# ml-rust/blazr

Measured on AMD Instinct MI355X. Metric: decode tokens/sec, Llama-3-8B AWQ-INT4 seq=1 on MI355X (and HBM-roofline fraction), higher is better.
Workload: dtype i4; 1 GPU; llama3-8b-awq greedy decode, batch 1, seq=1, prompt 16 (seed 26), whole step as one hipGraph; N>1 = independent replicas; resident_weight_bytes=5754585088, context_at_end=242

## Files before the change

### blazr_amd/csrc/bz_kernels.hip

```cpp
#include "bz_internal.h"
#include "bz_dev.h"
#include "bz_ggml.h"
#include <math.h>

#include <hip/hip_ext.h>

static thread_local BzTimingSink* g_sink = nullptr;
void bzk_set_timing_sink(BzTimingSink* s) { g_sink = s; }
BzTimingSink* bzk_timing_sink() { return g_sink; }

template <int NTH>
__device__ __forceinline__ void zero_duty(long long* zb, int zn) {
  if (zb)
    for (int i = blockIdx.x * NTH + threadIdx.x; i < zn; i += gridDim.x * NTH) zb[i] = 0;
}

template <int FIX>
__device__ __forceinline__ float vget(const void* p, int i, int act) {
  if (FIX) return round_act(fix2f(((const long long*)p)[i], act), act);
  return ((const float*)p)[i];
}

template <int FIX> struct RawT { typedef float T; };
template <> struct RawT<1> { typedef long long T; };
// ... 274 lines not shown
static size_t mlp_smem(int H) { return (size_t)(H >> 5) * XQ_NP * 16 + (size_t)(H >> 7) * 32 + 16 * 128 * 8 + 2 * XQ_NP * 16 + 32 + 16 * 8 + 64; }

bool bzk_mlp_fusable(const LinearDev& gu, const LinearDev& dn, int H, int I) {
  return gu.kind == LK_Q4G && dn.kind == LK_Q4G && !gu.perm && !dn.perm && gu.N == 2 * I && gu.K == H && dn.N == H && dn.K == I &&
         (H == 2048 || H == 4096) && I % 128 == 0 && mlp_smem(H) <= 64 * 1024;
}

int bzk_mlp_q4g(hipStream_t s, const LinearDev& gu, const LinearDev& dn, int H, int I, const Pro& pro, long long* acc, long long* zero_buf, int zero_n) {
  if (!bzk_mlp_fusable(gu, dn, H, I) || pro.act != BZ_F16) BZ_FAIL(BZ_E_INVALID, "fused MLP does not apply to this shape / activation dtype");
  const size_t smem = mlp_smem(H);
  const double bytes = (double)gu.algo_bytes + (double)dn.algo_bytes;
#define LAUNCH_MLP(FIX, GP, TP, W_) BZ_LAUNCH("mlp_q4g<norm+gate/up+silu+down>", bytes, (k_mlp_q4g<FIX, GP, TP, W_, BZ_F16>), dim3(I / 64), dim3(W_ * 64), smem, s, \
    (const uint4*)gu.w, (const __half*)gu.scales, (const unsigned char*)gu.zeros, gu.bias, (const uint4*)dn.w, (const __half*)dn.scales,            \
    (const unsigned char*)dn.zeros, dn.bias, H, I, pro, acc, zero_buf, zero_n)
  if (H == 4096) { if (pro.src.fix) LAUNCH_MLP(1, 2, 4, 16); else LAUNCH_MLP(0, 2, 4, 16); }
  else { if (pro.src.fix) LAUNCH_MLP(1, 2, 4, 8); else LAUNCH_MLP(0, 2, 4, 8); }
#undef LAUNCH_MLP
  BZ_HIP(hipGetLastError());
  return BZ_OK;
}

template <int MODE, int FIX, int MAXJ, int NPF>
__global__ __launch_bounds__(256) void k_gemv_q4g(const uint4* __restrict__ W, const __half* __restrict__ S,
                                                  const unsigned char* __restrict__ Z, const float* __restrict__ bias, int N, int K,
                                                  int GW, int nst, Pro pro, long long* acc, long long* zero_buf, int zero_n) {
  extern __shared__ __attribute__((aligned(16))) char smem[];
  const int KR = GW * 128;
  float* xs = (float*)smem;
  uint4* xpl = (uint4*)(xs + KR);
  int4* gpar = (int4*)(xpl + (KR >> 5) * XQ_NP);
  __half* sS = (__half*)(gpar + 2 * GW);
  unsigned char* sZ = (unsigned char*)(sS + 4 * GW * 64);
  float* red = (float*)(sZ + 4 * GW * 64);

  const int st = blockIdx.x % nst, ks = blockIdx.x / nst;
  const int wave = __builtin_amdgcn_readfirstlane(threadIdx.x >> 6), lane = threadIdx.x & 63;
  const int nt = st * 4 + wave;
  const bool wave_on = nt * 64 < N;
  const int G = K >> 7;
  const int k0 = ks * KR, g0 = ks * GW;

  zero_duty<256>(zero_buf, zero_n);

  const int ntc = wave_on ? nt : 0;
  unsigned sreg[8], zreg[4];
  {
    const unsigned* Sg = (const unsigned*)(S + ((size_t)ntc * G + g0) * 64);
    const unsigned* Zg = (const unsigned*)(Z + ((size_t)ntc * G + g0) * 64);
#pragma unroll
    for (int j = 0; j < 8; j++) sreg[j] = Sg[min(lane + 64 * j, GW * 32 - 1)];
#pragma unroll
    for (int j = 0; j < 4; j++) zreg[j] = Zg[min(lane + 64 * j, GW * 16 - 1)];
  }

  XRegs<MODE, FIX, MAXJ, Q4G_E> xr;
  xload<MODE, FIX, MAXJ, Q4G_E>(pro, k0, KR, xr);
  __builtin_amdgcn_sched_barrier(0);

  const uint4* wp = W + ((size_t)ntc * (K >> 5) + (k0 >> 5)) * 64 + lane;
  uint4 Wb[NPF][4];
#pragma unroll
  for (int b = 0; b < NPF; b++) {
    const int bc = min(b, GW - 1);
#pragma unroll
    for (int c = 0; c < 4; c++) Wb[b][c] = ldnt(wp + (bc * 4 + c) * 64);
  }

  xfinish<MODE, FIX, MAXJ, Q4G_E>(pro, KR, xr, xs, red, blockIdx.x == 0);
  {
    unsigned* sSw = (unsigned*)(sS + wave * GW * 64);
    unsigned* sZw = (unsigned*)(sZ + wave * GW * 64);
#pragma unroll
    for (int j = 0; j < 8; j++) if (lane + 64 * j < GW * 32) sSw[lane + 64 * j] = sreg[j];
#pragma unroll
    for (int j = 0; j < 4; j++) if (lane + 64 * j < GW * 16) sZw[lane + 64 * j] = zreg[j];
  }
  quant_x128<256>(xs, KR, xpl, gpar);
  __syncthreads();
  if (!wave_on) return;

  double y = 0.0;
  for (int gb = 0; gb < GW; gb += NPF) {
#pragma unroll
    for (int b = 0; b < NPF; b++) {
      const int g = gb + b;
      if (g < GW) {
        const float s = __half2float(sS[(wave * GW + g) * 64 + lane]);
        const int z = sZ[(wave * GW + g) * 64 + lane];
        q4g_consume(Wb[b], g, xpl, gpar, s, z, y);
        if (g + NPF < GW) {
#pragma unroll
          for (int c = 0; c < 4; c++) Wb[b][c] = ldnt(wp + ((g + NPF) * 4 + c) * 64);
        }
      }
    }
  }
  const int n = nt * 64 + lane;
  if (bias != nullptr && ks == 0) y += (double)bias[n];
  atomicAdd((unsigned long long*)(acc + n), (unsigned long long)d2fix(y, pro.act));
}

template <int FIX, int NJ, int ACT>
__global__ __launch_bounds__(768) void k_gemv_q4g_slim(const uint4* __restrict__ W, const __half* __restrict__ S, const unsigned char* __restrict__ Z,
                                                      const float* __restrict__ bias, int N, int H, Pro pro, long long* acc, long long* zero_buf, int zero_n) {
  __shared__ uint4 xpl[8 * XQ_NP];
  __shared__ int4 gpar[4];
  __shared__ double red[4];
  __shared__ unsigned cntv[2];
  volatile unsigned* cnt = cntv;
  const int tid = threadIdx.x, wave = __builtin_amdgcn_readfirstlane(tid >> 6), lane = tid & 63;
  const bool prolog = wave < 4;
  const int NKS = H >> 8, G = H >> 7;
  const int ksl = blockIdx.x % NKS, tg = blockIdx.x / NKS;
  asm volatile("" :: "s"(zero_buf), "s"(zero_n), "s"(acc), "s"(pro.h_in), "s"(pro.src.p), "s"(pro.norm_w), "s"(pro.h_out), "s"(pro.H),
               "s"(H), "s"(N), "s"(W), "s"(S), "s"(Z), "s"(bias));
  if (tid == 0) { cnt[0] = 0; cnt[1] = 0; }
  if (prolog) {
    const int pt = tid;
    const bool hasprev = pro.src.p != nullptr;
    const void* prevp = hasprev ? pro.src.p : (const void*)pro.h_in;
    float4 ha[NJ], hb[NJ];
    typename RawT<FIX>::T pv[NJ][8];
#pragma unroll
    for (int j = 0; j < NJ; j++) {
      const int i0 = (j * 256 + pt) * 8;
      ha[j] = *(const float4*)(pro.h_in + i0); hb[j] = *(const float4*)(pro.h_in + i0 + 4);
#pragma unroll
      for (int e = 0; e < 8; e++) pv[j][e] = vraw<FIX>(prevp, (FIX || hasprev) ? i0 + e : 0);
    }
    const int osl = 32 * ksl, jsel = osl >> 8, p0 = osl & 255;
    const bool mine = pt >= p0 && pt < p0 + 32;
    const int so = min(max(pt - p0, 0), 31);
    const float4 na = *(const float4*)(pro.norm_w + (osl + so) * 8), nb = *(const float4*)(pro.norm_w + (osl + so) * 8 + 4);
    __builtin_amdgcn_sched_barrier(0);
    __syncthreads();
    __builtin_amdgcn_sched_barrier(0);
    float v[NJ][8];
    double ssd = 0.0;
#pragma unroll
    for (int j = 0; j < NJ; j++) {
      const float t[8] = {ha[j].x, ha[j].y, ha[j].z, ha[j].w, hb[j].x, hb[j].y, hb[j].z, hb[j].w};
#pragma unroll
      for (int e = 0; e < 8; e++) v[j][e] = hasprev ? round_t<ACT>(t[e] + round_t<ACT>(FIX ? fix2f((long long)pv[j][e], ACT) : (float)pv[j][e])) : t[e];
#pragma unroll
      for (int e = 0; e < 8; e += 2) ssd += (double)(v[j][e] * v[j][e]) + (double)(v[j][e + 1] * v[j][e + 1]);
      if (blockIdx.x == 0 && pro.h_out) {
        const int i0 = (j * 256 + pt) * 8;
        *(float4*)(pro.h_out + i0) = make_float4(v[j][0], v[j][1], v[j][2], v[j][3]); *(float4*)(pro.h_out + i0 + 4) = make_float4(v[j][4], v[j][5], v[j][6], v[j][7]);
      }
    }
    ssd = wave_sum_d(ssd);
    if (lane == 0) { red[wave] = ssd; __builtin_amdgcn_s_waitcnt(0xc07f); atomicAdd((unsigned*)&cnt[0], 1u); }
    if (p0 / 64 == wave) {
      lds_wait_count(&cnt[0], 4);
      const float ss = (float)((red[0] + red[1]) + (red[2] + red[3]));
      const float rs = rms_scale(ss, (float)H, pro.eps);
      float sv[8];
#pragma unroll
      for (int e = 0; e < 8; e++) {
        sv[e] = v[0][e];
#pragma unroll
        for (int j = 1; j < NJ; j++) sv[e] = (j == jsel) ? v[j][e] : sv[e];
      }
      const float nwv[8] = {na.x, na.y, na.z, na.w, nb.x, nb.y, nb.z, nb.w};
      float x[8];
      float am = 0.f;
#pragma unroll
      for (int e = 0; e < 8; e++) { x[e] = mine ? round_t<ACT>(nwv[e] * round_t<ACT>(sv[e] * rs)) : 0.f; am = fmaxf(am, fabsf(x[e])); }
      am = grp_reduce<16, OpMax>(am);
      unsigned w[XQ_NP]; int sp[XQ_NP]; float cs;
      xq_split8(x, am, w, sp, cs);
#pragma unroll
      for (int p = 0; p < XQ_NP; p++) sp[p] = grp_reduce<16, OpAdd>(sp[p]);
      const int4 g2w = xq_gpar_hi<16>(w, sp);
      if (mine) {
        unsigned* plw = (unsigned*)xpl + ((so >> 2) * XQ_NP) * 4 + (so & 3);
#pragma unroll
        for (int p = 0; p < XQ_NP; p++) plw[p * 4] = w[p];
        if ((so & 15) == 0) {
          gpar[2 * (so >> 4)] = make_int4(__float_as_int(cs), sp[0], sp[1], sp[2]);
          gpar[2 * (so >> 4) + 1] = g2w;
        }
      }
      __builtin_amdgcn_s_waitcnt(0xc07f);
      if (lane == 0) atomicAdd((unsigned*)&cnt[1], 1u);
    }
    return;
  }
  const int tq = tg * 8 + (wave - 4);
  const bool q_on = tq * 64 < N;
  const int tqc = q_on ? tq : 0;
  const uint4* wq = W + ((size_t)tqc * (H >> 5) + ksl * 8) * 64 + lane;
  uint4 Q[8]; float sq[2]; int zq[2];
  __syncthreads();
  __builtin_amdgcn_sched_barrier(0);
#pragma unroll
  for (int c = 0; c < 8; c++) Q[c] = ldnt(wq + c * 64);
#pragma unroll
  for (int b = 0; b < 2; b++) { const size_t ix = ((size_t)tqc * G + ksl * 2 + b) * 64 + lane; sq[b] = __half2float(S[ix]); zq[b] = Z[ix]; }
  if (zero_buf)
    for (int i = blockIdx.x * 512 + (tid - 256); i < zero_n; i += gridDim.x * 512) zero_buf[i] = 0;
  lds_wait_count(&cnt[1], 1);
  if (q_on) {
    double y = 0.0;
#pragma unroll
    for (int b = 0; b < 2; b++) {
      if (b == 0) q4g_consume_at<0, 4>(Q, 0, 0, xpl, gpar, sq[0], zq[0], y);
      else q4g_consume_at<4, 4>(Q, 4, 2, xpl, gpar, sq[1], zq[1], y);
    }
    const int n = tq * 64 + lane;
    if (bias != nullptr && ksl == 0) y += (double)bias[n];
    atomicAdd((unsigned long long*)(acc + n), (unsigned long long)d2fix(y, ACT));
  }
}

template <int XDT>
__global__ __launch_bounds__(512) void k_gemm_q4g_rows(const uint4* __restrict__ W, const __half* __restrict__ S, const unsigned char* __restrict__ Z,
                                                      const float* __restrict__ bias, int N, int K, const unsigned short* __restrict__ X, int rows,
                                                      long long* __restrict__ acc) {
  __shared__ __attribute__((aligned(16))) float xs[8 * 256];
  __shared__ uint4 xpl[8 * 8 * XQ_NP];
  __shared__ int4 gpar[8 * 4];
  const int tid = threadIdx.x, wave = __builtin_amdgcn_readfirstlane(tid >> 6), lane = tid & 63;
  const int NKS = K >> 8, G = K >> 7;
  const int ksl = blockIdx.x % NKS, tq = (blockIdx.x / NKS) * 8 + wave;
  const bool q_on = tq * 64 < N;
  const int tqc = q_on ? tq : 0;
  const int xr = tid >> 6;
  const uint2 xraw = *(const uint2*)(X + (size_t)min(xr, rows - 1) * K + ksl * 256 + lane * 4);
  __builtin_amdgcn_sched_barrier(0);
  uint4 Q[2][4]; float sq[2]; int zq[2];
  {
    const uint4* wq = W + ((size_t)tqc * (K >> 5) + ksl * 8) * 64 + lane;
#pragma unroll
    for (int b = 0; b < 2; b++)
#pragma unroll
      for (int c = 0; c < 4; c++) Q[b][c] = ldnt(wq + (b * 4 + c) * 64);
#pragma unroll
    for (int b = 0; b < 2; b++) { const size_t ix = ((size_t)tqc * G + ksl * 2 + b) * 64 + lane; sq[b] = __half2float(S[ix]); zq[b] = Z[ix]; }
  }
  {
    const unsigned u[2] = {xraw.x, xraw.y};
    float v[4];
#pragma unroll
    for (int i = 0; i < 2; i++) {
      if (XDT == BZ_F16) { v[2 * i] = __half2float(__ushort_as_half((unsigned short)(u[i] & 0xffffu))); v[2 * i + 1] = __half2float(__ushort_as_half((unsigned short)(u[i] >> 16))); }
      else { v[2 * i] = __uint_as_float(u[i] << 16); v[2 * i + 1] = __uint_as_float(u[i] & 0xffff0000u); }
    }
    const bool on = xr < rows;
    *(float4*)(xs + xr * 256 + lane * 4) = on ? make_float4(v[0], v[1], v[2], v[3]) : make_float4(0.f, 0.f, 0.f, 0.f);
  }
  __syncthreads();
  quant_x128<512>(xs, 8 * 256, xpl, gpar);
  __syncthreads();
  if (!q_on) return;
  const int n = tq * 64 + lane;
  const double bv = (bias != nullptr && ksl == 0) ? (double)bias[n] : 0.0;
#pragma unroll
  for (int r = 0; r < 8; r++) {
    if (r < rows) {
      double y = bv;
      q4g_consume(Q[0], r * 2, xpl, gpar, sq[0], zq[0], y);
      q4g_consume(Q[1], r * 2 + 1, xpl, gpar, sq[1], zq[1], y);
      atomicAdd((unsigned long long*)(acc + (size_t)r * N + n), (unsigned long long)d2fix(y, XDT));
    }
  }
}

__global__ void k_fix_rows_finish(long long* acc, size_t n, int act, float* out) {
  for (size_t i = (size_t)blockIdx.x * blockDim.x + threadIdx.x; i < n; i += (size_t)gridDim.x * blockDim.x) { out[i] = round_act(fix2f(acc[i], act), act); acc[i] = 0; }
}

bool bzk_gemm_q4g_rows_ok(const LinearDev& L) { return L.kind == LK_Q4G && !L.perm && L.K % 256 == 0 && L.N % 64 == 0; }

int bzk_gemm_q4g_rows(hipStream_t s, const LinearDev& L, int xdt, const void* x16, int rows, int act, long long* acc, float* y) {
  if (!bzk_gemm_q4g_rows_ok(L) || (xdt != BZ_F16 && xdt != BZ_BF16) || xdt != act) BZ_FAIL(BZ_E_UNSUPPORTED, "gemm_q4g_rows: unsupported weight / activation format");
  const int nks = L.K / 256, ntg = (L.N / 64 + 7) / 8;
  for (int r0 = 0; r0 < rows; r0 += 8) {
    const int nr = std::min(8, rows - r0);
    const unsigned short* xp = (const unsigned short*)x16 + (size_t)r0 * L.K;
    const double bytes = (double)L.algo_bytes;
    if (xdt == BZ_F16) BZ_LAUNCH("gemm_q4g_rows", bytes, k_gemm_q4g_rows<BZ_F16>, dim3(nks * ntg), dim3(512), 0, s, (const uint4*)L.w, (const __half*)L.scales,
                                 (const unsigned char*)L.zeros, L.bias, L.N, L.K, xp, nr, acc);
    else BZ_LAUNCH("gemm_q4g_rows", bytes, k_gemm_q4g_rows<BZ_BF16>, dim3(nks * ntg), dim3(512), 0, s, (const uint4*)L.w, (const __half*)L.scales,
                   (const unsigned char*)L.zeros, L.bias, L.N, L.K, xp, nr, acc);
    hipLaunchKernelGGL(k_fix_rows_finish, dim3(std::min<size_t>(1024, ((size_t)nr * L.N + 255) / 256)), dim3(256), 0, s, acc, (size_t)nr * L.N, act, y + (size_t)r0 * L.N);
  }
  BZ_HIP(hipGetLastError());
  return BZ_OK;
}

bool bzk_gemv_slim_ok(const LinearDev& L, const Pro& pro) {
  static const bool off = getenv("BZ_NO_SLIM_QKV") != nullptr;
  return !off && L.kind == LK_Q4G && !L.perm && pro.mode == PRO_NORM && pro.perm == nullptr && L.K == pro.H && (L.K == 2048 || L.K == 4096 || L.K == 8192) && L.N % 64 == 0 &&
         L.N <= 16384;
}

enum { GQ_Q80 = 0, GQ_Q4K = 1, GQ_Q6K = 2, GQ_MIX = 3, GQ_Q5K = 4, GQ_Q40 = 5, GQ_Q41 = 6, GQ_Q50 = 7, GQ_Q51 = 8 };
__host__ __device__ constexpr bool gq_legacy(int f) { return f == GQ_Q40 || f == GQ_Q41 || f == GQ_Q50 || f == GQ_Q51; }
__host__ __device__ constexpr bool gq_has5(int f) { return f == GQ_Q50 || f == GQ_Q51; }
__host__ __device__ constexpr bool gq_affine(int f) { return f == GQ_Q41 || f == GQ_Q51; }
#define XQ_MAX 8355000.0f

template <int FMT>
__device__ __forceinline__ void quant8_x32(const float (&v)[8], int e0, bool on, int lane, unsigned* xh, unsigned* xm, unsigned* xl, int4* cpar, int4* cpar6 = nullptr) {
  float am = 0.f;
#pragma unroll
  for (int i = 0; i < 8; i++) am = fmaxf(am, fabsf(v[i]));
  am = grp_reduce<4, OpMax>(am);
  const float inv = am > 0.f ? XQ_MAX / am : 0.f;
  unsigned wh[2] = {0, 0}, wm[2] = {0, 0}, wl[2] = {0, 0};
  int sa[3] = {0, 0, 0}, sb[3] = {0, 0, 0};
  int ta[3] = {0, 0, 0}, tb[3] = {0, 0, 0};
#pragma unroll
  for (int i = 0; i < 8; i++) {
    const int xi = (int)rintf(v[i] * inv);
    const int lo = ((xi + 128) & 255) - 128;
    const int r1 = (xi - lo) >> 8;
    const int mid = ((r1 + 128) & 255) - 128;
    const int hi = (r1 - mid) >> 8;
    wh[i >> 2] |= ((unsigned)hi & 255u) << (8 * (i & 3));
    wm[i >> 2] |= ((unsigned)mid & 255u) << (8 * (i & 3));
    wl[i >> 2] |= ((unsigned)lo & 255u) << (8 * (i & 3));
    if (FMT == GQ_Q4K || FMT == GQ_MIX) { sa[0] += hi; sa[1] += mid; sa[2] += lo; if (i >= 4) { sb[0] += hi; sb[1] += mid; sb[2] += lo; } }
    if (FMT == GQ_Q6K || FMT == GQ_Q5K || gq_legacy(FMT)) { sa[0] += hi; sa[1] += mid; sa[2] += lo; }
  }
  if (FMT == GQ_Q6K || FMT == GQ_MIX) {
    const bool second = (lane & 2) != 0;
#pragma unroll
    for (int q = 0; q < 3; q++) {
      const int mine = sa[q] + dpp_get<DPP_XOR1>(sa[q]);
      const int other = dpp_get<DPP_XOR2>(mine);
      ta[q] = second ? other : mine;
      tb[q] = second ? mine : other;
    }
    if (FMT == GQ_Q6K) {
#pragma unroll
      for (int q = 0; q < 3; q++) { sa[q] = ta[q]; sb[q] = tb[q]; }
    }
  }
  if (FMT == GQ_Q4K || FMT == GQ_MIX) {
#pragma unroll
    for (int q = 0; q < 3; q++) {
      sa[q] = grp_reduce<4, OpAdd>(sa[q]);
      sb[q] = grp_reduce<4, OpAdd>(sb[q]);
    }
  }
  if (FMT == GQ_Q5K || gq_legacy(FMT)) {
#pragma unroll
    for (int q = 0; q < 3; q++) sa[q] = grp_reduce<4, OpAdd>(sa[q]);
  }
  if (on) {
    *(uint2*)(xh + e0 / 4) = make_uint2(wh[0], wh[1]);
    *(uint2*)(xm + e0 / 4) = make_uint2(wm[0], wm[1]);
    *(uint2*)(xl + e0 / 4) = make_uint2(wl[0], wl[1]);
    if ((lane & 3) == 0) {
      cpar[2 * (e0 >> 5)] = make_int4(__float_as_int(am * (1.0f / XQ_MAX)), sa[0], sa[1], sa[2]);
      cpar[2 * (e0 >> 5) + 1] = make_int4(sb[0], sb[1], sb[2], 0);
      if (FMT == GQ_MIX) {
        cpar6[2 * (e0 >> 5)] = make_int4(__float_as_int(am * (1.0f / XQ_MAX)), ta[0], ta[1], ta[2]);
        cpar6[2 * (e0 >> 5) + 1] = make_int4(tb[0], tb[1], tb[2], 0);
      }
// ... 2019 lines not shown

template <int HD, int KVDT, int WIN = 0>
__global__ __launch_bounds__(256) void k_attn_decode(AttnArgs a) {
  extern __shared__ __attribute__((aligned(16))) char smem[];
  constexpr int half = HD / 2;
  constexpr int LDR = HD + 4;
  const int rep = a.nq / a.nkv;
  float* qs = (float*)smem;
  float* knew = qs + HD;
  float* vnew = knew + HD;
  float* wred = vnew + HD;
  float* ored = wred + 8;
  const int hq = blockIdx.x, kvh = hq / rep;
  const int tid = threadIdx.x, wave = __builtin_amdgcn_readfirstlane(tid >> 6), lane = tid & 63;
  const int pos = a.pos[0];
  const int len = a.q_only ? pos : pos + 1;
  const int ncache = pos;
  const int lo = WIN ? att_lo(len, a.window) : 0;
  const KvView& kv = a.kv;
  zero_duty<256>(a.zero_buf, a.zero_n);

  if (!a.q_only) {
    const float* cr = a.cos_t + (size_t)pos * half;
    const float* sr = a.sin_t + (size_t)pos * half;
    for (int idx = tid; idx < 2 * half; idx += 256) {
      const int hh = idx / half, i = idx % half;
      const int base = hh == 0 ? hq * HD : a.nq * HD + kvh * HD;
      const int ia = a.interleaved ? 2 * i : i, ib = a.interleaved ? 2 * i + 1 : i + half;
      const float x0 = vsrc_get(a.qkv, base + ia, a.act), x1 = vsrc_get(a.qkv, base + ib, a.act);
      const float c = cr[i], s = sr[i];
      const float y0 = round_act(rope_lo(x0, x1, c, s), a.act), y1 = round_act(rope_hi(x0, x1, c, s), a.act);
      if (hh == 0) { qs[ia] = y0; qs[ib] = y1; }
      else { knew[ia] = y0; knew[ib] = y1; }
    }
    for (int i = tid; i < HD; i += 256) vnew[i] = vsrc_get(a.qkv, a.nq * HD + a.nkv * HD + kvh * HD + i, a.act);
    __syncthreads();
    if (hq % rep == 0) {
      size_t woff;
      if (kv.paged) woff = kv_slot_off(kv, a.layer, kvh, kv.slot ? kv.slot[0] : (kv.block_table[pos / kv.bs] * kv.bs + pos % kv.bs));
      else woff = kv_row_off(kv, a.layer, kvh, pos);
      for (int i = tid; i < HD; i += 256) { kv_st(kv.k, woff + i, kv.dtype, knew[i]); kv_st(kv.v, woff + i, kv.dtype, vnew[i]); }
    }
  } else {
    for (int i = tid; i < HD; i += 256) qs[i] = ((const float*)a.qkv.p)[hq * HD + i];
    __syncthreads();
  }

  const float scale = div_rn(1.0f, sqrt_rn((float)HD));
  float m = -INFINITY, l = 0.f;
  float o[HD];
#pragma unroll
  for (int i = 0; i < HD; i++) o[i] = 0.f;
  for (int p = lo + tid; p < len; p += 256) {
    KvRow<HD, KVDT> kr, vr;
    const size_t ro = p < ncache ? kv_row_off(kv, a.layer, kvh, p) : 0;
    if (p < ncache) kr.load(kv.k, ro); else kr.from_f32(knew);
    if (KVDT != BZ_F32) { if (p < ncache) vr.load(kv.v, ro); else vr.from_f32(vnew); }
    float d = 0.f;
#pragma unroll
    for (int i = 0; i < HD; i += 4) {
      const float4 qa = *(const float4*)(qs + i);
      d += kr.get(i) * qa.x + kr.get(i + 1) * qa.y + kr.get(i + 2) * qa.z + kr.get(i + 3) * qa.w;
    }
    if (KVDT == BZ_F32) { if (p < ncache) vr.load(kv.v, ro); else vr.from_f32(vnew); }
    const float s = d * scale;
    if (m == -INFINITY) {
      m = s; l = 1.f;
#pragma unroll
      for (int i = 0; i < HD; i++) o[i] = vr.get(i);
    } else {
      const float mn = fmaxf(m, s);
      const float alpha = bz_expf(m - mn), e = bz_expf(s - mn);
      l = l * alpha + e;
      m = mn;
#pragma unroll
      for (int i = 0; i < HD; i++) o[i] = o[i] * alpha + e * vr.get(i);
    }
  }
  const float wm = wave_max(m);
  if (lane == 0) wred[wave] = wm;
  __syncthreads();
  const float M = fmaxf(fmaxf(wred[0], wred[1]), fmaxf(wred[2], wred[3]));
  const float w = (m == -INFINITY) ? 0.f : bz_expf(m - M);
  const float ws = wave_sum(l * w);
  if (lane == 0) wred[4 + wave] = ws;
  const int nrows = min(len - lo, 256);
  if (tid < nrows) {
#pragma unroll
    for (int i = 0; i < HD; i += 4) *(float4*)(ored + tid * LDR + i) = make_float4(o[i] * w, o[i + 1] * w, o[i + 2] * w, o[i + 3] * w);
  }
  __syncthreads();
  const float inv = div_rn(1.0f, (wred[4] + wred[5]) + (wred[6] + wred[7]));
  constexpr int PH = 256 / HD;
  const int col = tid % HD, ph = tid / HD;
  float acc = 0.f;
  for (int r = ph; r < nrows; r += PH) acc += ored[r * LDR + col];
  __syncthreads();
  ored[ph * LDR + col] = acc;
  __syncthreads();
  if (tid < HD) {
    float t = 0.f;
#pragma unroll
    for (int q = 0; q < PH; q++) t += ored[q * LDR + tid];
    a.out[(size_t)hq * HD + tid] = round_act(t * inv, a.act);
  }
}


template <int KVDT, int FUSE, int TPW, int NW, int PAGED, int HD = 128, int WIN = 0>
__global__ __launch_bounds__(NW * 64) void k_attn2(AttnArgs a, const uint4* __restrict__ W, const __half* __restrict__ S,
                                               const unsigned char* __restrict__ Z, const float* __restrict__ bias, int CS, long long* acc) {
  static_assert(HD == 128 || (HD == 64 && FUSE != 1), "head_dim 128, or 64 without the int4 o_proj");
  constexpr int half = HD / 2, NPC = HD / 8, RPL = 64 / NPC, PW = 256 / NW, NL = PW / RPL, OW = NW > 8 ? 8 : NW, NTH = NW * 64;
  asm volatile("" :: "s"(a.zero_buf), "s"(a.zero_n), "s"(a.kv.k), "s"(a.kv.v), "s"(a.kv.cap), "s"(a.kv.layer_stride), "s"(a.layer), "s"(a.act),
               "s"(a.interleaved), "s"(a.rope_cur), "s"(a.qkv.p), "s"(a.qkv.fix), "s"(a.nq), "s"(a.nkv), "s"(a.q_only), "s"(a.pos), "s"(W), "s"(S),
               "s"(Z), "s"(bias), "s"(CS), "s"(acc), "s"(a.out), "s"(a.kv.bs), "s"(a.kv.n_kv));
  extern __shared__ __attribute__((aligned(16))) char smem[];
  unsigned* q2 = (unsigned*)smem;
  unsigned* k2 = q2 + 64;
  unsigned* v2 = k2 + 64;
  double* pout = (double*)(v2 + 64);
  double* lred = pout + NW * 128;
  float* wred = (float*)(lred + NW);
  float* outh = wred + 2 * NW;
  uint4* xpl = (uint4*)(outh + 128);
  int4* gpar = (int4*)(xpl + 4 * XQ_NP);
  const int rep = a.nq / a.nkv;
  const int hq = FUSE ? blockIdx.x / CS : blockIdx.x, cs = FUSE ? blockIdx.x % CS : 0, kvh = hq / rep;
  const int tid = threadIdx.x, wave = __builtin_amdgcn_readfirstlane(tid >> 6), lane = tid & 63;
  const int piece = lane % NPC, rsub = lane / NPC;
  const KvView& kv = a.kv;
  const int pos_v = a.pos[0];
  const int slot_v = PAGED ? *(kv.slot ? kv.slot : a.pos) : 0;
  const int fixq = a.q_only ? 0 : a.qkv.fix;
  int i0, i1;
  {
    const int hh = tid / half, i = tid % half;
    const int base = hh == 0 ? hq * HD : a.nq * HD + kvh * HD;
    const int ia = a.interleaved ? 2 * i : i, ib = a.interleaved ? 2 * i + 1 : i + half;
    const int vb = a.nq * HD + a.nkv * HD + kvh * HD + 2 * i;
    i0 = hh < 2 ? base + ia : vb; i1 = hh < 2 ? base + ib : vb + 1;
    if (a.q_only) { i0 = hq * HD + 2 * i; i1 = i0 + 1; }
    if (hh > 2) { i0 = 0; i1 = 0; }
  }
  unsigned r0l, r0h, r1l, r1h;
  vsrc_issue(a.qkv.p, fixq, i0, r0l, r0h);
  vsrc_issue(a.qkv.p, fixq, i1, r1l, r1h);
  const float* rc = a.q_only ? (const float*)a.qkv.p : a.rope_cur;
  const float pc = rc[tid % half], ps = rc[half + tid % half];
  if (a.zero_buf) {
    const int nblk = FUSE ? a.nq * CS : a.nq;
    for (int i = blockIdx.x * NTH + tid; i < a.zero_n; i += nblk * NTH) a.zero_buf[i] = 0;
  }
  uint4 Wb[FUSE == 1 ? TPW : 1][4];
  const int t0 = (cs * OW + wave % OW) * TPW;
  constexpr int DLD = FUSE == 2 ? TPW : 1;
  uint4 Wd[DLD];
  const int nd0 = (cs * NW + wave) * DLD * RPL;
  if (FUSE == 2) {
    const int K = a.nq * HD;
    const unsigned short* wd = (const unsigned short*)W;
#pragma unroll
    for (int t = 0; t < DLD; t++) Wd[t] = ldnt((const uint4*)(wd + (size_t)(nd0 + t * RPL + rsub) * K + hq * HD + piece * 8));
  }
  if (FUSE == 1) {
    const int K = a.nq * HD;
#pragma unroll
    for (int t = 0; t < TPW; t++) {
      const uint4* wp = W + ((size_t)(t0 + t) * (K >> 5) + hq * 4) * 64 + lane;
#pragma unroll
      for (int c = 0; c < 4; c++) Wb[t][c] = ldnt(wp + c * 64);
    }
  }
  __builtin_amdgcn_sched_barrier(0);
  const int pos = __builtin_amdgcn_readfirstlane(pos_v);
  const int pmax = pos > 0 ? pos - 1 : 0;
  const int len = a.q_only ? pos : pos + 1;
  const int lo = WIN ? att_lo(len, a.window) : 0, cb = WIN ? (lo & ~255) : 0;
  const unsigned short* kb0 = (const unsigned short*)kv.k + (size_t)a.layer * kv.layer_stride;
  const unsigned short* vb0 = (const unsigned short*)kv.v + (size_t)a.layer * kv.layer_stride;
  uint4 kr[NL], vr[NL];
#pragma unroll
  for (int i = 0; i < NL; i++) { kr[i] = make_uint4(0, 0, 0, 0); vr[i] = make_uint4(0, 0, 0, 0); }
#define ATT_ROW(i) (((i) * NW + wave) * RPL + rsub)
#define ATT_LIVE(c0_, i) ((c0_) + ((i) * NW + wave) * RPL < len)
  if (cb + wave * RPL < len) {
    if (!PAGED) {
      const unsigned short* kb = kb0 + (size_t)kvh * kv.cap * HD;
      const unsigned short* vb = vb0 + (size_t)kvh * kv.cap * HD;
#pragma unroll
      for (int i = 0; i < NL; i++) {
        if (ATT_LIVE(cb, i)) {
          const unsigned off = (unsigned)min(cb + ATT_ROW(i), pmax) * HD + piece * 8;
          kr[i] = *(const uint4*)(kb + off);
          vr[i] = *(const uint4*)(vb + off);
        }
      }
    } else {
      int blk[NL];
#pragma unroll
      for (int i = 0; i < NL; i++) blk[i] = ATT_LIVE(cb, i) ? kv.block_table[min(cb + ATT_ROW(i), pmax) / kv.bs] : 0;
#pragma unroll
      for (int i = 0; i < NL; i++) {
        if (ATT_LIVE(cb, i)) {
          const int pp = min(cb + ATT_ROW(i), pmax);
          const size_t off = (((size_t)blk[i] * kv.n_kv + kvh) * kv.bs + (pp % kv.bs)) * HD + piece * 8;
          kr[i] = *(const uint4*)(kb0 + off);
          vr[i] = *(const uint4*)(vb0 + off);
        }
      }
    }
  }
  const float px0 = vsrc_finish(fixq, r0l, r0h, a.act), px1 = vsrc_finish(fixq, r1l, r1h, a.act);
  if (!a.q_only) {
    if (tid < 2 * half) {
      const int hh = tid / half, i = tid % half;
      const int ia = a.interleaved ? 2 * i : i, ib = a.interleaved ? 2 * i + 1 : i + half;
      const float y0 = round_act(rope_lo(px0, px1, pc, ps), a.act), y1 = round_act(rope_hi(px0, px1, pc, ps), a.act);
      unsigned short* dst = (unsigned short*)(hh == 0 ? q2 : k2);
      const unsigned p0 = pack2<KVDT>(y0, y1);
      dst[ia] = (unsigned short)(p0 & 0xffffu);
      dst[ib] = (unsigned short)(p0 >> 16);
    } else if (tid < 3 * half) {
      v2[tid - 2 * half] = pack2<KVDT>(px0, px1);
    }
    __syncthreads();
    if (hq % rep == 0 && cs == 0 && tid < half) {
      size_t woff;
      if (PAGED) woff = kv_slot_off(kv, a.layer, kvh, kv.slot ? slot_v : (kv.block_table[pos / kv.bs] * kv.bs + pos % kv.bs));
      else woff = kv_row_off_t<0>(kv, a.layer, kvh, pos);
      ((unsigned*)((unsigned short*)kv.k + woff))[tid] = k2[tid];
      ((unsigned*)((unsigned short*)kv.v + woff))[tid] = v2[tid];
    }
  } else {
    if (tid < half) q2[tid] = pack2<KVDT>(px0, px1);
    __syncthreads();
  }

  const float scale = div_rn(1.0f, sqrt_rn((float)HD));
  const uint4 qq = ((const uint4*)q2)[piece];
  float qf[8];
  unpack2<KVDT>(qq.x, qf[0], qf[1]); unpack2<KVDT>(qq.y, qf[2], qf[3]); unpack2<KVDT>(qq.z, qf[4], qf[5]); unpack2<KVDT>(qq.w, qf[6], qf[7]);
  const bool single = len - cb <= 256;
  float sc_[NL];
  float Mw = -INFINITY;
#define ATT_SCORES(c0_)                                                                                                    \
  _Pragma("unroll") for (int i = 0; i < NL; i++) {                                                                         \
    if (!ATT_LIVE(c0_, i)) { sc_[i] = -INFINITY; continue; }                                                               \
    const int p = (c0_) + ATT_ROW(i);                                                                                      \
    uint4 kk = kr[i];                                                                                                      \
    if (!a.q_only && p == pos) { kk = ((const uint4*)k2)[piece]; vr[i] = ((const uint4*)v2)[piece]; }                      \
    float kf[8];                                                                                                           \
    unpack2<KVDT>(kk.x, kf[0], kf[1]); unpack2<KVDT>(kk.y, kf[2], kf[3]); unpack2<KVDT>(kk.z, kf[4], kf[5]); unpack2<KVDT>(kk.w, kf[6], kf[7]); \
    double d = 0.0;                                                                                                        \
    _Pragma("unroll") for (int e = 0; e < 8; e++) d = fma((double)kf[e], (double)qf[e], d);                                \
    d = grp_sum_d<NPC>(d);                                                                                                 \
    sc_[i] = (p < len && (!WIN || p >= lo)) ? (float)d * scale : -INFINITY;                                                \
  }
  for (int c0 = cb; c0 < len; c0 += 256) {
    const bool won = c0 + wave * RPL < len;
    if (!won) continue;
    if (c0 > cb) {
#pragma unroll
      for (int i = 0; i < NL; i++)
        if (ATT_LIVE(c0, i)) kr[i] = *(const uint4*)(kb0 + kv_row_off_t<PAGED>(kv, 0, kvh, min(c0 + ATT_ROW(i), pmax)) + piece * 8);
    }
    ATT_SCORES(c0)
#pragma unroll
    for (int i = 0; i < NL; i++) Mw = fmaxf(Mw, sc_[i]);
  }
  Mw = wave_max(Mw);
  if (lane == 0) wred[wave] = Mw;
  __syncthreads();
  float Mall = wred[0];
#pragma unroll
  for (int w = 1; w < NW; w++) Mall = fmaxf(Mall, wred[w]);
  double accv[8] = {0.0, 0.0, 0.0, 0.0, 0.0, 0.0, 0.0, 0.0};
  double lsum = 0.0;
  for (int c0 = cb; c0 < len; c0 += 256) {
    const bool won = c0 + wave * RPL < len;
    if (!won) continue;
    if (!single) {
#pragma unroll
      for (int i = 0; i < NL; i++) {
        if (ATT_LIVE(c0, i)) {
          const size_t off = kv_row_off_t<PAGED>(kv, 0, kvh, min(c0 + ATT_ROW(i), pmax)) + piece * 8;
          kr[i] = *(const uint4*)(kb0 + off);
          vr[i] = *(const uint4*)(vb0 + off);
        }
      }
      ATT_SCORES(c0)
    }
#pragma unroll
    for (int i = 0; i < NL; i++) {
      if (!ATT_LIVE(c0, i)) continue;
      const float e = (sc_[i] == -INFINITY) ? 0.f : bz_expf(sc_[i] - Mall);
      const double ed = (double)e;
      lsum += ed;
      float v[8];
      unpack2<KVDT>(vr[i].x, v[0], v[1]); unpack2<KVDT>(vr[i].y, v[2], v[3]);
      unpack2<KVDT>(vr[i].z, v[4], v[5]); unpack2<KVDT>(vr[i].w, v[6], v[7]);
#pragma unroll
      for (int q = 0; q < 8; q++) accv[q] = fma(ed, (double)v[q], accv[q]);
    }
  }
#undef ATT_SCORES
#undef ATT_LIVE
#undef ATT_ROW
  if (NPC == 8) lsum += dpp_get<DPP_ROR8>(lsum);
  lsum = xrow32_d(xrow16_d(lsum));
#pragma unroll
  for (int q = 0; q < 8; q++) {
    if (NPC == 8) accv[q] += dpp_get<DPP_ROR8>(accv[q]);
    accv[q] = xrow32_d(xrow16_d(accv[q]));
  }
  if (lane < NPC) {
#pragma unroll
    for (int q = 0; q < 8; q++) pout[wave * HD + piece * 8 + q] = accv[q];
  }
  if (lane == 0) lred[wave] = lsum;
  __syncthreads();
  float Orun = 0.f, Lrun = 1.f;
  if (tid < HD) {
    double oc = 0.0, Lc = 0.0;
#pragma unroll
    for (int w = 0; w < NW; w++) { oc += pout[w * HD + tid]; Lc += lred[w]; }
    Orun = (float)oc; Lrun = (float)Lc;
  }
  if (!FUSE) {
    if (tid < HD) a.out[(size_t)hq * HD + tid] = round_act(div_rn(Orun, Lrun), a.act);
    return;
  }
  if (tid < HD) outh[tid] = round_act(div_rn(Orun, Lrun), a.act);
  if (FUSE == 2) {
    __syncthreads();
    const float4 oa = *(const float4*)(outh + piece * 8), ob = *(const float4*)(outh + piece * 8 + 4);
    const float of8[8] = {oa.x, oa.y, oa.z, oa.w, ob.x, ob.y, ob.z, ob.w};
#pragma unroll
    for (int t = 0; t < DLD; t++) {
      float w8[8];
      unpack2<KVDT>(Wd[t].x, w8[0], w8[1]); unpack2<KVDT>(Wd[t].y, w8[2], w8[3]); unpack2<KVDT>(Wd[t].z, w8[4], w8[5]); unpack2<KVDT>(Wd[t].w, w8[6], w8[7]);
      double d = 0.0;
#pragma unroll
      for (int e = 0; e < 8; e++) d += (double)__fmul_rn(w8[e], of8[e]);
      d = grp_sum_d<NPC>(d);
      const int n = nd0 + t * RPL + rsub;
      if (piece == 0) {
        if (bias != nullptr && hq == 0) d += (double)bias[n];
        atomicAdd((unsigned long long*)(acc + n), (unsigned long long)d2fix(d, a.act));
      }
    }
    return;
  }
  float sc[FUSE == 1 ? TPW : 1]; int zp[FUSE == 1 ? TPW : 1];
  {
    const int G = (a.nq * HD) >> 7;
#pragma unroll
    for (int t = 0; t < (FUSE == 1 ? TPW : 1); t++) {
      sc[t] = __half2float(S[((size_t)(t0 + t) * G + hq) * 64 + lane]);
      zp[t] = Z[((size_t)(t0 + t) * G + hq) * 64 + lane];
    }
  }
  __syncthreads();
  quant_x128<NW * 64>(outh, HD, xpl, gpar);
  __syncthreads();
#pragma unroll
  for (int t = 0; t < (FUSE == 1 ? TPW : 1); t++) {
    double y = 0.0;
    q4g_consume(Wb[t], 0, xpl, gpar, sc[t], zp[t], y);
    const int n = (t0 + t) * 64 + lane;
    if (bias != nullptr && hq == 0) y += (double)bias[n];
    if (wave < OW) atomicAdd((unsigned long long*)(acc + n), (unsigned long long)d2fix(y, a.act));
  }
}


template <int PAGED, int FUSE = 0, int WIN = 0>
__global__ __launch_bounds__(512) void k_attn2f(AttnArgs a, const uint4* __restrict__ Wq, const uint4* __restrict__ Hd, const float* __restrict__ bias, int CS, long long* acc) {
  constexpr int HD = 128, half = 64, NW = 8, PW = 256 / NW, NL = PW / 4, NTH = NW * 64;
  __shared__ __attribute__((aligned(16))) float qf[HD], kf[HD], vf[HD];
  __shared__ float wred[2 * NW];
  __shared__ __attribute__((aligned(16))) float pout[NW * 128];
  __shared__ __attribute__((aligned(16))) float outh[FUSE ? HD : 4];
  __shared__ __attribute__((aligned(16))) unsigned xh[FUSE ? 32 : 4], xm[FUSE ? 32 : 4], xl[FUSE ? 32 : 4];
  __shared__ int4 cpar[FUSE ? 8 : 1];
  asm volatile("" :: "s"(a.zero_buf), "s"(a.zero_n), "s"(a.kv.k), "s"(a.kv.v), "s"(a.kv.cap), "s"(a.kv.layer_stride), "s"(a.layer), "s"(a.act),
               "s"(a.interleaved), "s"(a.rope_cur), "s"(a.qkv.p), "s"(a.qkv.fix), "s"(a.nq), "s"(a.nkv), "s"(a.q_only), "s"(a.pos), "s"(a.out),
               "s"(a.kv.bs), "s"(a.kv.n_kv), "s"(Wq), "s"(Hd), "s"(bias), "s"(CS), "s"(acc));
  const int rep = a.nq / a.nkv;
  const int hq = FUSE ? blockIdx.x / CS : blockIdx.x, cs = FUSE ? blockIdx.x % CS : 0, kvh = hq / rep;
  const int tid = threadIdx.x, wave = __builtin_amdgcn_readfirstlane(tid >> 6), lane = tid & 63;
  const int piece = lane & 15, rsub = lane >> 4;
  const KvView& kv = a.kv;
  const int pos_v = a.pos[0];
  const int slot_v = PAGED ? *(kv.slot ? kv.slot : a.pos) : 0;
  const int fixq = a.q_only ? 0 : a.qkv.fix;
  int i0, i1;
  {
    const int hh = tid / half, i = tid % half;
    const int base = hh == 0 ? hq * HD : a.nq * HD + kvh * HD;
    const int ia = a.interleaved ? 2 * i : i, ib = a.interleaved ? 2 * i + 1 : i + half;
    const int vb = a.nq * HD + a.nkv * HD + kvh * HD + 2 * i;
    i0 = hh < 2 ? base + ia : vb; i1 = hh < 2 ? base + ib : vb + 1;
    if (a.q_only) { i0 = hq * HD + 2 * i; i1 = i0 + 1; }
    if (hh > 2) { i0 = 0; i1 = 0; }
  }
  unsigned r0l, r0h, r1l, r1h;
  vsrc_issue(a.qkv.p, fixq, i0, r0l, r0h);
  vsrc_issue(a.qkv.p, fixq, i1, r1l, r1h);
  const float* rc = a.q_only ? (const float*)a.qkv.p : a.rope_cur;
  const float pc = rc[tid % half], ps = rc[half + tid % half];
  if (a.zero_buf)
    for (int i = blockIdx.x * NTH + tid; i < a.zero_n; i += (FUSE ? a.nq * CS : a.nq) * NTH) a.zero_buf[i] = 0;
  uint4 Wb[4]; uint4 hdw = make_uint4(0, 0, 0, 0);
  const int t0 = cs * NW + wave;
  if (FUSE) {
    const int K = a.nq * HD;
    const uint4* wp = Wq + ((size_t)t0 * (K >> 5) + hq * 4) * 64 + lane;
#pragma unroll
    for (int c = 0; c < 4; c++) Wb[c] = ldnt(wp + c * 64);
    hdw = Hd[((size_t)t0 * (K >> 8) + (hq >> 1)) * 64 + lane];
  }
  __builtin_amdgcn_sched_barrier(0);
  const int pos = __builtin_amdgcn_readfirstlane(pos_v);
  const int pmax = pos > 0 ? pos - 1 : 0;
  const int len = a.q_only ? pos : pos + 1;
  const int lo = WIN ? att_lo(len, a.window) : 0, cb = WIN ? (lo & ~255) : 0;
  const float* kb0 = (const float*)kv.k + (size_t)a.layer * kv.layer_stride;
  const float* vb0 = (const float*)kv.v + (size_t)a.layer * kv.layer_stride;
  float4 kr[NL][2], vr[NL][2];
#pragma unroll
  for (int i = 0; i < NL; i++) { kr[i][0] = kr[i][1] = vr[i][0] = vr[i][1] = make_float4(0.f, 0.f, 0.f, 0.f); }
#define ATF_ROW(i) (((i) * NW + wave) * 4 + rsub)
#define ATF_LIVE(c0_, i) ((c0_) + ((i) * NW + wave) * 4 < len)
  if (cb + wave * 4 < len) {
#pragma unroll
    for (int i = 0; i < NL; i++) {
      if (ATF_LIVE(cb, i)) {
        const size_t off = kv_row_off_t<PAGED>(kv, 0, kvh, min(cb + ATF_ROW(i), pmax)) + piece * 8;
        kr[i][0] = *(const float4*)(kb0 + off); kr[i][1] = *(const float4*)(kb0 + off + 4);
        vr[i][0] = *(const float4*)(vb0 + off); vr[i][1] = *(const float4*)(vb0 + off + 4);
      }
    }
  }
  const float px0 = vsrc_finish(fixq, r0l, r0h, a.act), px1 = vsrc_finish(fixq, r1l, r1h, a.act);
  if (!a.q_only) {
    if (tid < 2 * half) {
      const int hh = tid / half, i = tid % half;
      const int ia = a.interleaved ? 2 * i : i, ib = a.interleaved ? 2 * i + 1 : i + half;
      float* dst = hh == 0 ? qf : kf;
      dst[ia] = round_act(rope_lo(px0, px1, pc, ps), a.act);
      dst[ib] = round_act(rope_hi(px0, px1, pc, ps), a.act);
    } else if (tid < 2 * half + 64) {
      vf[2 * (tid - 2 * half)] = px0; vf[2 * (tid - 2 * half) + 1] = px1;
    }
    __syncthreads();
    if (hq % rep == 0 && cs == 0 && tid < HD) {
      size_t woff;
      if (PAGED) woff = kv_slot_off(kv, a.layer, kvh, kv.slot ? slot_v : (kv.block_table[pos / kv.bs] * kv.bs + pos % kv.bs));
      else woff = kv_row_off_t<0>(kv, a.layer, kvh, pos);
      ((float*)kv.k)[woff + tid] = kf[tid];
      ((float*)kv.v)[woff + tid] = vf[tid];
    }
  } else {
    if (tid < 64) { qf[2 * tid] = px0; qf[2 * tid + 1] = px1; }
    __syncthreads();
  }
  const float scale = div_rn(1.0f, sqrt_rn((float)HD));
  const float4 qa = *(const float4*)(qf + piece * 8), qb = *(const float4*)(qf + piece * 8 + 4);
  float Mrun = -INFINITY, Lrun = 0.f, Orun = 0.f;
  for (int c0 = cb; c0 < len; c0 += 256) {
    const bool won = c0 + wave * 4 < len;
    if (c0 > cb) {
      __syncthreads();
      if (won) {
#pragma unroll
        for (int i = 0; i < NL; i++) {
          if (ATF_LIVE(c0, i)) {
            const size_t off = kv_row_off_t<PAGED>(kv, 0, kvh, min(c0 + ATF_ROW(i), pmax)) + piece * 8;
            kr[i][0] = *(const float4*)(kb0 + off); kr[i][1] = *(const float4*)(kb0 + off + 4);
            vr[i][0] = *(const float4*)(vb0 + off); vr[i][1] = *(const float4*)(vb0 + off + 4);
          }
        }
      }
    }
    float sc_[NL];
    float mloc = -INFINITY;
    if (won) {
#pragma unroll
      for (int i = 0; i < NL; i++) {
        if (!ATF_LIVE(c0, i)) { sc_[i] = -INFINITY; continue; }
        const int p = c0 + ATF_ROW(i);
        float4 k0 = kr[i][0], k1 = kr[i][1];
        if (!a.q_only && p == pos) {
          k0 = *(const float4*)(kf + piece * 8); k1 = *(const float4*)(kf + piece * 8 + 4);
          vr[i][0] = *(const float4*)(vf + piece * 8); vr[i][1] = *(const float4*)(vf + piece * 8 + 4);
        }
        float d = k0.x * qa.x + k0.y * qa.y + k0.z * qa.z + k0.w * qa.w + k1.x * qb.x + k1.y * qb.y + k1.z * qb.z + k1.w * qb.w;
        d = grp_reduce<16, OpAdd>(d);
        sc_[i] = (p < len && (!WIN || p >= lo)) ? d * scale : -INFINITY;
        mloc = fmaxf(mloc, sc_[i]);
      }
      mloc = wave_max(mloc);
    }
    if (lane == 0) wred[wave] = mloc;
    __syncthreads();
    float Mc = wred[0];
#pragma unroll
    for (int w = 1; w < NW; w++) Mc = fmaxf(Mc, wred[w]);
    float accv[8] = {0.f, 0.f, 0.f, 0.f, 0.f, 0.f, 0.f, 0.f};
    float lsum = 0.f;
    if (won) {
#pragma unroll
      for (int i = 0; i < NL; i++) {
        if (!ATF_LIVE(c0, i)) continue;
// ... 2022 lines not shown
```

Baseline: 699.2 tokens/s.

## Reorder loads in fused rmsnorm-GEMM and attention-Wo kernels to overlap latency

In the fused norm+q4 GEMM kernel, the scale and zero-point loads are now issued as raw loads before the weight loads and before the LDS counter wait, and the two group-consume calls are separated by a scheduling barrier. The LDS waits switch to a ds-only variant. In the FUSE==1 attention kernel, all K rows are loaded before any V rows, and the Wo weight, scale and zero-point loads move after the KV loads. The current-position V override moves into the accumulation loop. The aim is to get the latency-critical loads issued first and let the weight loads overlap attention work, at the cost of longer register lifetimes and more complex load ordering.

```diff
diff --git a/blazr_amd/csrc/bz_kernels.hip b/blazr_amd/csrc/bz_kernels.hip
--- a/blazr_amd/csrc/bz_kernels.hip
+++ b/blazr_amd/csrc/bz_kernels.hip
@@ -450,7 +450,7 @@
     ssd = wave_sum_d(ssd);
     if (lane == 0) { red[wave] = ssd; __builtin_amdgcn_s_waitcnt(0xc07f); atomicAdd((unsigned*)&cnt[0], 1u); }
     if (p0 / 64 == wave) {
-      lds_wait_count(&cnt[0], 4);
+      lds_wait_count_ds(&cnt[0], 4);
       const float ss = (float)((red[0] + red[1]) + (red[2] + red[3]));
       const float rs = rms_scale(ss, (float)H, pro.eps);
       float sv[8];
@@ -492,20 +492,22 @@
   uint4 Q[8]; float sq[2]; int zq[2];
   __syncthreads();
   __builtin_amdgcn_sched_barrier(0);
-#pragma unroll
-  for (int c = 0; c < 8; c++) Q[c] = ldnt(wq + c * 64);
-#pragma unroll
-  for (int b = 0; b < 2; b++) { const size_t ix = ((size_t)tqc * G + ksl * 2 + b) * 64 + lane; sq[b] = __half2float(S[ix]); zq[b] = Z[ix]; }
   if (zero_buf)
     for (int i = blockIdx.x * 512 + (tid - 256); i < zero_n; i += gridDim.x * 512) zero_buf[i] = 0;
-  lds_wait_count(&cnt[1], 1);
+  unsigned short sqr[2]; unsigned char zqr[2];
+#pragma unroll
+  for (int b = 0; b < 2; b++) { const size_t ix = ((size_t)tqc * G + ksl * 2 + b) * 64 + lane; sqr[b] = ((const unsigned short*)S)[ix]; zqr[b] = Z[ix]; }
+#pragma unroll
+  for (int c = 0; c < 8; c++) Q[c] = ldnt(wq + c * 64);
+  __builtin_amdgcn_sched_barrier(0);
+  lds_wait_count_ds(&cnt[1], 1);
+#pragma unroll
+  for (int b = 0; b < 2; b++) { sq[b] = __half2float(__ushort_as_half(sqr[b])); zq[b] = zqr[b]; }
   if (q_on) {
     double y = 0.0;
-#pragma unroll
-    for (int b = 0; b < 2; b++) {
-      if (b == 0) q4g_consume_at<0, 4>(Q, 0, 0, xpl, gpar, sq[0], zq[0], y);
-      else q4g_consume_at<4, 4>(Q, 4, 2, xpl, gpar, sq[1], zq[1], y);
-    }
+    q4g_consume_at<0, 4>(Q, 0, 0, xpl, gpar, sq[0], zq[0], y);
+    __builtin_amdgcn_sched_barrier(0);
+    q4g_consume_at<4, 4>(Q, 4, 2, xpl, gpar, sq[1], zq[1], y);
     const int n = tq * 64 + lane;
     if (bias != nullptr && ksl == 0) y += (double)bias[n];
     atomicAdd((unsigned long long*)(acc + n), (unsigned long long)d2fix(y, ACT));
@@ -2831,8 +2833,6 @@
     const int nblk = FUSE ? a.nq * CS : a.nq;
     for (int i = blockIdx.x * NTH + tid; i < a.zero_n; i += nblk * NTH) a.zero_buf[i] = 0;
   }
-  uint4 Wb[FUSE == 1 ? TPW : 1][4];
-  const int t0 = (cs * OW + wave % OW) * TPW;
   constexpr int DLD = FUSE == 2 ? TPW : 1;
   uint4 Wd[DLD];
   const int nd0 = (cs * NW + wave) * DLD * RPL;
@@ -2841,15 +2841,6 @@
     const unsigned short* wd = (const unsigned short*)W;
 #pragma unroll
     for (int t = 0; t < DLD; t++) Wd[t] = ldnt((const uint4*)(wd + (size_t)(nd0 + t * RPL + rsub) * K + hq * HD + piece * 8));
-  }
-  if (FUSE == 1) {
-    const int K = a.nq * HD;
-#pragma unroll
-    for (int t = 0; t < TPW; t++) {
-      const uint4* wp = W + ((size_t)(t0 + t) * (K >> 5) + hq * 4) * 64 + lane;
-#pragma unroll
-      for (int c = 0; c < 4; c++) Wb[t][c] = ldnt(wp + c * 64);
-    }
   }
   __builtin_amdgcn_sched_barrier(0);
   const int pos = __builtin_amdgcn_readfirstlane(pos_v);
@@ -2858,6 +2849,7 @@
   const int lo = WIN ? att_lo(len, a.window) : 0, cb = WIN ? (lo & ~255) : 0;
   const unsigned short* kb0 = (const unsigned short*)kv.k + (size_t)a.layer * kv.layer_stride;
   const unsigned short* vb0 = (const unsigned short*)kv.v + (size_t)a.layer * kv.layer_stride;
+  constexpr bool KFIRST = FUSE == 1;
   uint4 kr[NL], vr[NL];
 #pragma unroll
   for (int i = 0; i < NL; i++) { kr[i] = make_uint4(0, 0, 0, 0); vr[i] = make_uint4(0, 0, 0, 0); }
@@ -2872,8 +2864,13 @@
         if (ATT_LIVE(cb, i)) {
           const unsigned off = (unsigned)min(cb + ATT_ROW(i), pmax) * HD + piece * 8;
           kr[i] = *(const uint4*)(kb + off);
-          vr[i] = *(const uint4*)(vb + off);
+          if (!KFIRST) vr[i] = *(const uint4*)(vb + off);
         }
+      }
+      if (KFIRST) {
+#pragma unroll
+        for (int i = 0; i < NL; i++)
+          if (ATT_LIVE(cb, i)) vr[i] = *(const uint4*)(vb + (unsigned)min(cb + ATT_ROW(i), pmax) * HD + piece * 8);
       }
     } else {
       int blk[NL];
@@ -2885,10 +2882,33 @@
           const int pp = min(cb + ATT_ROW(i), pmax);
           const size_t off = (((size_t)blk[i] * kv.n_kv + kvh) * kv.bs + (pp % kv.bs)) * HD + piece * 8;
           kr[i] = *(const uint4*)(kb0 + off);
-          vr[i] = *(const uint4*)(vb0 + off);
+          if (!KFIRST) vr[i] = *(const uint4*)(vb0 + off);
         }
       }
-    }
+      if (KFIRST) {
+#pragma unroll
+        for (int i = 0; i < NL; i++)
+          if (ATT_LIVE(cb, i)) vr[i] = *(const uint4*)(vb0 + (((size_t)blk[i] * kv.n_kv + kvh) * kv.bs + (min(cb + ATT_ROW(i), pmax) % kv.bs)) * HD + piece * 8);
+      }
+    }
+  }
+  uint4 Wb[FUSE == 1 ? TPW : 1][4];
+  const int t0 = (cs * OW + wave % OW) * TPW;
+  unsigned short sraw[FUSE == 1 ? TPW : 1] = {}; unsigned char zraw[FUSE == 1 ? TPW : 1] = {};
+  if (FUSE == 1) {
+    const int K = a.nq * HD, G = K >> 7;
+#pragma unroll
+    for (int t = 0; t < TPW; t++) {
+      sraw[t] = ((const unsigned short*)S)[((size_t)(t0 + t) * G + hq) * 64 + lane];
+      zraw[t] = Z[((size_t)(t0 + t) * G + hq) * 64 + lane];
+    }
+#pragma unroll
+    for (int t = 0; t < TPW; t++) {
+      const uint4* wp = W + ((size_t)(t0 + t) * (K >> 5) + hq * 4) * 64 + lane;
+#pragma unroll
+      for (int c = 0; c < 4; c++) Wb[t][c] = ldnt(wp + c * 64);
+    }
+    __builtin_amdgcn_sched_barrier(0);
   }
   const float px0 = vsrc_finish(fixq, r0l, r0h, a.act), px1 = vsrc_finish(fixq, r1l, r1h, a.act);
   if (!a.q_only) {
@@ -2928,7 +2948,7 @@
     if (!ATT_LIVE(c0_, i)) { sc_[i] = -INFINITY; continue; }                                                               \
     const int p = (c0_) + ATT_ROW(i);                                                                                      \
     uint4 kk = kr[i];                                                                                                      \
-    if (!a.q_only && p == pos) { kk = ((const uint4*)k2)[piece]; vr[i] = ((const uint4*)v2)[piece]; }                      \
+    if (!a.q_only && p == pos) { kk = ((const uint4*)k2)[piece]; if (!KFIRST) vr[i] = ((const uint4*)v2)[piece]; }         \
     float kf[8];                                                                                                           \
     unpack2<KVDT>(kk.x, kf[0], kf[1]); unpack2<KVDT>(kk.y, kf[2], kf[3]); unpack2<KVDT>(kk.z, kf[4], kf[5]); unpack2<KVDT>(kk.w, kf[6], kf[7]); \
     double d = 0.0;                                                                                                        \
@@ -2965,8 +2985,13 @@
         if (ATT_LIVE(c0, i)) {
           const size_t off = kv_row_off_t<PAGED>(kv, 0, kvh, min(c0 + ATT_ROW(i), pmax)) + piece * 8;
           kr[i] = *(const uint4*)(kb0 + off);
-          vr[i] = *(const uint4*)(vb0 + off);
+          if (!KFIRST) vr[i] = *(const uint4*)(vb0 + off);
         }
+      }
+      if (KFIRST) {
+#pragma unroll
+        for (int i = 0; i < NL; i++)
+          if (ATT_LIVE(c0, i)) vr[i] = *(const uint4*)(vb0 + kv_row_off_t<PAGED>(kv, 0, kvh, min(c0 + ATT_ROW(i), pmax)) + piece * 8);
       }
       ATT_SCORES(c0)
     }
@@ -2976,9 +3001,11 @@
       const float e = (sc_[i] == -INFINITY) ? 0.f : bz_expf(sc_[i] - Mall);
       const double ed = (double)e;
       lsum += ed;
+      uint4 vv = vr[i];
+      if (KFIRST && !a.q_only && c0 + ATT_ROW(i) == pos) vv = ((const uint4*)v2)[piece];
       float v[8];
-      unpack2<KVDT>(vr[i].x, v[0], v[1]); unpack2<KVDT>(vr[i].y, v[2], v[3]);
-      unpack2<KVDT>(vr[i].z, v[4], v[5]); unpack2<KVDT>(vr[i].w, v[6], v[7]);
+      unpack2<KVDT>(vv.x, v[0], v[1]); unpack2<KVDT>(vv.y, v[2], v[3]);
+      unpack2<KVDT>(vv.z, v[4], v[5]); unpack2<KVDT>(vv.w, v[6], v[7]);
 #pragma unroll
       for (int q = 0; q < 8; q++) accv[q] = fma(ed, (double)v[q], accv[q]);
     }
@@ -3032,14 +3059,8 @@
     return;
   }
   float sc[FUSE == 1 ? TPW : 1]; int zp[FUSE == 1 ? TPW : 1];
-  {
-    const int G = (a.nq * HD) >> 7;
-#pragma unroll
-    for (int t = 0; t < (FUSE == 1 ? TPW : 1); t++) {
-      sc[t] = __half2float(S[((size_t)(t0 + t) * G + hq) * 64 + lane]);
-      zp[t] = Z[((size_t)(t0 + t) * G + hq) * 64 + lane];
-    }
-  }
+#pragma unroll
+  for (int t = 0; t < (FUSE == 1 ? TPW : 1); t++) { sc[t] = __half2float(__ushort_as_half(sraw[t])); zp[t] = zraw[t]; }
   __syncthreads();
   quant_x128<NW * 64>(outh, HD, xpl, gpar);
   __syncthreads();
```

New measurement: 705.9 tokens/s (median of 6 runs). No clear change (+1.0%).
